# MonsieurETM/QPSK

Measured on AMD Instinct MI355X. Metric: complex Msamples/s demodulated + % HBM roofline, 2400-baud RRC+Costas path, higher is better.
Workload: dtype f32

## Files before the change

qpsk_amd/csrc/api.cpp:

```cpp
#include "../../include/qpsk_hip.h"
#include "host_math.h"
#include "kernels.h"

#include <hip/hip_runtime.h>
#include <limits.h>
#include <math.h>
#include <stdarg.h>
#include <stdio.h>
#include <stdlib.h>
#include <string.h>
#include <time.h>
#include <algorithm>
#include <map>
#include <vector>

using namespace qpsk;

static thread_local char g_err[512] = "";

static int fail(int code, const char *fmt, ...)
{
    va_list ap;
    va_start(ap, fmt);
    vsnprintf(g_err, sizeof g_err, fmt, ap);
// ... 8 lines not shown
            return fail(QPSK_ERR_HIP, "%s: %s (%s:%d)", #expr, hipGetErrorString(e_), __FILE__, __LINE__); \
    } while (0)

#define KERNEL_TRY(expr)                                                                      \
    do {                                                                                      \
        (void)hipGetLastError();  \
        int e_ = (expr);                                                                      \
        if (e_ != 0)                                                                          \
            return fail(QPSK_ERR_HIP, "%s: %s (%s:%d)", #expr, hipGetErrorString((hipError_t)e_), __FILE__, __LINE__); \
    } while (0)

struct DevBuf {
    void *p = nullptr;
    size_t cap = 0;
};

struct Tuning {
    int fused_g = -1, fused_s = -1, fused_lds = -1;
    int generic = -1;
    int pipe_nf = -1;
    int pipe_v = -1, pipe_g = -1;
    int layout_lo = -1, layout_hi = -1;
    int pipe_variant = -1;
    int hist_generic = -1;
    int fir_generic = -1;
    int stream_scan = -1;
    int stream_poll = -1;
    int stream_block = -1;
    int stream_carrier = -1;
    int lean_dma = -1;
    int hist_onepass = -1;
    int est_waves = -1;
    int lean_pair = -1;
    int viterbi_lds = -1;
    int fft_fused = -1;
    int viterbi_chunk_rows = -1;
};

static const struct { const char *name; int Tuning::*field; } TUNING_KEYS[] = {
    {"QPSK_FUSED_G", &Tuning::fused_g},       {"QPSK_FUSED_S", &Tuning::fused_s},     {"QPSK_FUSED_LDS", &Tuning::fused_lds},
    {"QPSK_FUSED_GENERIC", &Tuning::generic}, {"QPSK_PIPE_NF", &Tuning::pipe_nf},
    {"QPSK_PIPE_DBG", &Tuning::pipe_variant}, {"QPSK_HIST_GENERIC", &Tuning::hist_generic},
    {"QPSK_PIPE_V", &Tuning::pipe_v},         {"QPSK_PIPE_G", &Tuning::pipe_g},
    {"QPSK_PIPE_LAYOUT_LO", &Tuning::layout_lo}, {"QPSK_PIPE_LAYOUT_HI", &Tuning::layout_hi},
    {"QPSK_FIR_GENERIC", &Tuning::fir_generic}, {"QPSK_FFT_FUSED", &Tuning::fft_fused},
    {"QPSK_STREAM_BLOCK", &Tuning::stream_block}, {"QPSK_STREAM_POLL", &Tuning::stream_poll},
    {"QPSK_STREAM_SCAN", &Tuning::stream_scan}, {"QPSK_STREAM_CARRIER", &Tuning::stream_carrier},
    {"QPSK_LEAN_DMA", &Tuning::lean_dma},     {"QPSK_LEAN_PAIR", &Tuning::lean_pair},
    {"QPSK_EST_WAVES", &Tuning::est_waves},   {"QPSK_HIST_ONEPASS", &Tuning::hist_onepass},
    {"QPSK_VITERBI_LDS", &Tuning::viterbi_lds},   {"QPSK_VITERBI_CHUNK_ROWS", &Tuning::viterbi_chunk_rows},
};

#ifdef QPSK_PIPE_PROFILE
static const int PIPE_VARIANT_MASK = ~0;
#else
static const int PIPE_VARIANT_MASK = 4 | 8 | 16 | 64 | 128 | 256 | 512 | 1024 | 8192;
#endif

struct qpsk_ctx {
    int device = 0;
    Tuning tune;
    int ncu = 256;
    const char *last_kernel = "";
    int viterbi_launches = 0;
    bool taps_symmetric = false;
    hipStream_t stream = nullptr;
    qpsk_params prm{};
    int cycles = 0, nsym = 0;
    float taps[QPSK_NTAPS];
    float damping = 0.f, alpha = 0.f, beta = 0.f;
    float min_freq = 0.f, max_freq = 0.f;
    float *d_taps = nullptr;
    float *d_gains = nullptr;
    unsigned *h_done = nullptr, *d_done = nullptr;
    unsigned done_expect = 0;
    int *h_status = nullptr;
    int *d_status = nullptr;
    std::vector<float> h_gains;
    DevBuf index, filtered, mixed, keystream, sympad, mislist;
    DevBuf datacostas;
    DevBuf vitdec;
    DevBuf softgain;
// ... 512 lines not shown
            *d_index_out = (const int32_t *)c->index.p;
            return QPSK_OK;
        }
        const size_t bytes = sizeof(float) * 2 * (size_t)nframes * c->prm.frame_size;
        rc = ensure(c, c->filtered, bytes);
        if (rc) return rc;
        KERNEL_TRY(fir_full_rate(c, d_in, nullptr, (float *)c->filtered.p, nframes, c->prm.frame_size, pitch));
        KERNEL_TRY(launch_timing_hist((const float *)c->filtered.p, nframes, c->prm.frame_size, c->cycles,
                                      (int32_t *)c->index.p, nullptr, tuned(c->tune.hist_generic, 0) == 2, c->stream));
        *d_index_out = (const int32_t *)c->index.p;
        return QPSK_OK;
    }
    rc = fft_timing_indices(c, d_in, nframes, (int32_t *)c->index.p, nullptr, nullptr, pitch);
    if (rc) return rc;
    *d_index_out = (const int32_t *)c->index.p;
    return QPSK_OK;
}

struct ExtAcq {
    const int32_t *index;
    const float *seed;
};

static int rx_batch_common(qpsk_ctx *c, const float *d_in, long long frame_pitch, int nframes, int nbw, uint8_t *d_sym,
                           float *d_freq, float *d_phase, float *d_costas, int32_t *d_index, float *d_hz,
                           const ExtAcq *ext = nullptr, uint8_t *d_data = nullptr)
{
    if (!c || !d_in || !(d_sym || d_data)) return fail(QPSK_ERR_ARG, "qpsk_rx_batch: null context, input or symbol buffer");
    if (nframes <= 0) return fail(QPSK_ERR_ARG, "qpsk_rx_batch: nframes = %d", nframes);
    if (frame_pitch == 0) frame_pitch = c->prm.frame_size;
    if (frame_pitch < c->prm.frame_size)
        return fail(QPSK_ERR_ARG, "qpsk_rx_batch_pitched: frame_pitch %lld below frame_size %d", frame_pitch, c->prm.frame_size);
    if (bind(c)) return QPSK_ERR_HIP;
    const bool pipe_ok = c->cycles == pipe_cycles() && (c->prm.frame_size % 2) == 0 && (frame_pitch % 2) == 0 &&
                         ((uintptr_t)d_in % 16) == 0 && nbw * pipe_frames(1) <= 64 &&
                         tuned(c->tune.generic, 0) == 0;
    FusedArgs a{};
    a.x = reinterpret_cast<const float2 *>(d_in);
    a.frame_pitch = (size_t)frame_pitch;
    a.nframes = nframes;
    a.frame_size = c->prm.frame_size;
    a.cycles = c->cycles;
    a.nsym = c->nsym;
    pick_tiling(c, nframes, nbw, &a.G, &a.S);
    a.fixed_index = c->prm.fixed_index;
    a.dbg = tuned(c->tune.pipe_variant, 0) & PIPE_VARIANT_MASK;
    a.lean_dma = tuned(c->tune.lean_dma, 1) != 0;
    a.lean_twowin = tuned(c->tune.lean_dma, 1) != 2 ? 1 : 0;
    a.est_waves = tuned(c->tune.est_waves, 0);
    a.lean_pair = tuned(c->tune.lean_pair, 3);
    a.taps = c->d_taps;
    a.gains = c->d_gains;
    a.nbw = nbw;
    a.min_freq = c->min_freq;
    a.max_freq = c->max_freq;
    a.rs = c->prm.rs;
    a.sym = d_sym ? d_sym : d_data;
    a.data_rule = d_data && !d_sym;
    if (d_data && d_sym && !d_costas) {
        if (int rd = ensure(c, c->datacostas, sizeof(float2) * (size_t)nframes * (size_t)c->nsym)) return rd;
        d_costas = (float *)c->datacostas.p;
    }
    a.freq = d_freq;
    a.phase = d_phase;
    a.costas = reinterpret_cast<float2 *>(d_costas);
    a.hz = d_hz;
    a.status = c->d_status;
    const bool ext_index = ext && ext->index;
    if (ext && ext->seed) {
        a.state_in = ext->seed;
        a.seed_setters = 1;
    }

    enum { K_GENERIC, K_FUSED_PIPE, K_PIPE2, K_LEAN };
    struct Plan {
        int kind = K_GENERIC, nframes = 0, G = 0, nf = 0;
        unsigned long long layout = 0;
    };
    const int pipe_v = tuned(c->tune.pipe_v, nframes > 16 * c->ncu ? 2 : 1);
    auto plan_general = [&](int nfr, int pv, Plan *pl) -> int {
        pl->nframes = nfr;
        if (pipe_ok && pv == 2) {
            int G = (nfr + c->ncu - 1) / c->ncu;
            if (G > pipe2_max_frames()) G = pipe2_max_frames();
            G = tuned(c->tune.pipe_g, G);
            if (G > pipe2_max_frames()) G = pipe2_max_frames();
            if (G * nbw > 64) G = 64 / nbw;
            if (G < 1) G = 1;
            unsigned long long layout = 0;
            if (c->tune.layout_lo >= 0 || c->tune.layout_hi >= 0) {
                layout = ((unsigned long long)(unsigned)tuned(c->tune.layout_lo, 0) << 4) |
                         ((unsigned long long)(unsigned)tuned(c->tune.layout_hi, 0) << 24);
                int units = 0, nwin = 0;
                for (int w = 1; w < 16; w++) { const int cw = (int)((layout >> (4 * w)) & 15); units += cw; nwin += cw != 0; }
                if (units < 1 || (G + 1) / 2 != units || pipe2_lds_bytes(G, nwin, nbw) > (size_t)MAX_LDS_BYTES)
                    return fail(QPSK_ERR_ARG, "QPSK_PIPE_LAYOUT_*: %d units on %d waves do not match %d frames per workgroup", units, nwin, G);
            } else {
                for (;;) {
                    layout = pipe2_default_layout((G + 1) / 2);
                    int nwin = 0;
                    for (int w = 1; w < 16; w++) nwin += ((layout >> (4 * w)) & 15) != 0;
                    if (layout && pipe2_lds_bytes(G, nwin, nbw) <= (size_t)MAX_LDS_BYTES) break;
                    if (G == 1) return fail(QPSK_ERR_ARG, "pipeline geometry does not fit: %d loops per frame", nbw);
                    G--;
                }
            }
            pl->kind = K_PIPE2;
            pl->G = G;
            pl->layout = layout;
        } else if (pipe_ok) {
            auto fits = [&](int nf_) {
                return pipe_frames(nf_) * nbw <= 64 && pipe_lds_bytes(nf_, nbw) <= (size_t)MAX_LDS_BYTES;
            };
            const int full = pipe_max_nf();
            int nf = 1;
            while (nf < full && (long long)c->ncu * pipe_frames(nf) < nfr) nf++;
            nf = tuned(c->tune.pipe_nf, nf);
            if (nf < 1) nf = 1;
            if (nf > full) nf = full;
            while (nf > 1 && !fits(nf)) nf--;
            if (!fits(nf))
                return fail(QPSK_ERR_ARG, "pipeline geometry does not fit: nf %d, %d loops per frame", nf, nbw);
            pl->kind = K_FUSED_PIPE;
            pl->nf = nf;
        } else {
            pl->kind = K_GENERIC;
        }
        return QPSK_OK;
    };
    Plan main_pl, rem_pl;
    bool lean = false;
    if (pipe_ok && c->taps_symmetric && (pipe_v == 3 || c->tune.pipe_v < 0)) {
        int G = (nframes + c->ncu - 1) / c->ncu;
        G = tuned(c->tune.pipe_g, G);
        if (G > pipe2_max_frames()) G = pipe2_max_frames();
        G += G & 1;
        const bool wanted = pipe_v == 3 || G >= 4;
        unsigned long long layout = 0;
        if (c->tune.layout_lo >= 0 || c->tune.layout_hi >= 0)
            layout = ((unsigned long long)(unsigned)tuned(c->tune.layout_lo, 0) << 4) |
                     ((unsigned long long)(unsigned)tuned(c->tune.layout_hi, 0) << 24);
        else if (G >= 2)
// ... 67 lines not shown
    if (c->prm.timing_mode == QPSK_TIMING_FFT && !ext_index && rem_pl.nframes == 0 && nbw == 1 && tuned(c->tune.fft_fused, 1) != 0 &&
        c->prm.frame_size >= timing_fft_first() + timing_fft_nfft() &&
        ((main_pl.kind == K_FUSED_PIPE && main_pl.nf == pipe_max_nf() && !(tuned(c->tune.pipe_variant, 0) & (128 | 4))) ||
         (main_pl.kind == K_LEAN && lean_est_ok(a, main_pl.G, main_pl.layout)))) {
        int rt = fft_timing_tables(c, &est_tw, &est_cs);
        if (rt) return rt;
        fused_fft = true;
    }
    const int32_t *idx = nullptr;
    if (ext_index) {
        idx = ext->index;
    } else {
        int rc = timing_indices(c, d_in, (size_t)frame_pitch, nframes, &idx, fused_fft);
        if (rc) return rc;
    }
    a.index = idx;
    if (fused_fft) {
        a.est_tw = reinterpret_cast<const double2 *>(est_tw);
        a.est_cs = reinterpret_cast<const double2 *>(est_cs);
        a.index_out = d_index ? (int32_t *)c->index.p : nullptr;
        if (d_index) idx = (const int32_t *)c->index.p;
    }

    auto execute = [&](const FusedArgs &fa, const Plan &pl) -> int {
        if (fa.est_tw && !(pl.kind == K_FUSED_PIPE && pl.nf == pipe_max_nf()) && pl.kind != K_LEAN)
            return fail(QPSK_ERR_STATE, "internal: in-launch FFT timing estimate planned for a kernel that has none");
        if (fa.data_rule && pl.kind != K_LEAN)
            return fail(QPSK_ERR_STATE, "internal: data rule planned for a kernel that has none");
        switch (pl.kind) {
        case K_LEAN:
            KERNEL_TRY(launch_rx_lean(fa, pl.G, pl.layout, c->d_status, c->stream));
            c->last_kernel = fa.est_tw ? "rx_lean_kernel (FFT timing estimate inside the launch)" : "rx_lean_kernel";
            break;
        case K_PIPE2:
            KERNEL_TRY(launch_rx_pipe2(fa, pl.G, pl.layout, c->d_status, c->stream));
            c->last_kernel = "rx_pipe2_kernel";
            break;
        case K_FUSED_PIPE:
            KERNEL_TRY(launch_rx_fused_pipe(fa, pl.nf, c->d_status, c->stream));
            c->last_kernel = fa.est_tw ? "rx_fused_pipe_kernel (FFT timing estimate inside the launch)" : "rx_fused_pipe_kernel";
            break;
        default:
            KERNEL_TRY(launch_rx_fused(fa, c->stream));
            c->last_kernel = "rx_fused_kernel";
        }
        return QPSK_OK;
    };
    {
        FusedArgs am = a;
        am.nframes = main_pl.nframes;
        int rc2 = execute(am, main_pl);
        if (rc2) return rc2;
        if (rem_pl.nframes > 0) {
            FusedArgs ar = a;
            const size_t o = (size_t)main_pl.nframes;
            ar.nframes = rem_pl.nframes;
            ar.x += o * a.frame_pitch;
            if (ar.index) ar.index += o;
            if (ar.state_in) ar.state_in += 2 * o * (size_t)nbw;
            ar.sym += o * (size_t)a.nsym;
            if (ar.freq) ar.freq += o;
            if (ar.phase) ar.phase += o;
            if (ar.hz) ar.hz += o;
            const char *lk = c->last_kernel;
            rc2 = execute(ar, rem_pl);
            if (rc2) return rc2;
            c->last_kernel = lk;
        }
    }
    if (hist_mode && !ext && c->d_hint && idx && tuned(c->tune.hist_onepass, -1) != 0) {
// ... 1314 lines not shown
```

qpsk_amd/csrc/kernels.h:

```cpp
#ifndef QPSK_KERNELS_H
#define QPSK_KERNELS_H

#include <hip/hip_runtime.h>
#include <stddef.h>
#include <stdint.h>

namespace qpsk {

constexpr int LOOKBACK = 128;
constexpr int LOOKAHEAD = 8;
constexpr int MAX_LDS_BYTES = 160 * 1024;
constexpr int MAX_INDEX = 7;
constexpr int STATUS_PIPE_TIMEOUT = 1;
constexpr int STATUS_PHASE_RANGE = 2;
constexpr int STATUS_NONFINITE = 3;
constexpr int STATUS_BAD_INDEX = 4;
constexpr int STATUS_EST_NONFINITE = 5;
constexpr int STATUS_SOFT_NONFINITE = 6;
constexpr int STATUS_SOFT_BAD_LAG = 7;

struct FusedArgs {
    const float2 *x;
    size_t frame_pitch;
    int nframes, frame_size, cycles, nsym;
    int G, S;
    int mixed;
    int share_simd0;
    const int32_t *index;
    int fixed_index;
    const double2 *est_tw, *est_cs;
    int32_t *index_out;
    int lean_twowin;
    int lean_dma;
    int est_waves;
    int lean_pair;
    int dbg;
    const float2 *dsrc;
    int dstride;
    const float2 *refill;
    float2 *refill_dst;
    int refill_planar;
    const int32_t *frame_list, *frame_list_count;
    const float *taps;
    const float *gains;
    int nbw;
    float min_freq, max_freq;
    double rs;
    const float *state_in;
    int seed_setters;
    float *state_out;
    uint8_t *sym;
    uint8_t *sym_pad;
    float *freq, *phase;
    float2 *costas;
    float *hz;
    int *status;
    float *carrier_state;
    float2 *carrier_tab;
    int carrier_frame;
    int data_rule;
};

size_t fused_lds_bytes(int G, int S, int cycles, int nbw);
int prepare_kernels(void);
int launch_rx_fused(const FusedArgs &a, hipStream_t s);
size_t pipe_lds_bytes(int NF, int nbw);
int pipe_frames(int NF);
int pipe_cycles(void);
int pipe_max_nf(void);
int prepare_pipe_kernel(void);
int launch_rx_fused_pipe(const FusedArgs &a, int NF, int *status, hipStream_t s);
int launch_costas_pipe(const FusedArgs &a, int NF, int *status, hipStream_t s);
size_t pipe2_lds_bytes(int G, int nwin, int nbw);
int pipe2_max_fir(void);
int pipe2_max_frames(void);
int pipe2_max_units_per_wave(void);
int pipe2_max_hw_waves(void);
unsigned long long pipe2_default_layout(int NU);
int launch_rx_pipe2(const FusedArgs &a, int G, unsigned long long layout, int *status, hipStream_t s);
size_t lean_lds_bytes(int G, int nwin);
unsigned long long lean_default_layout(int NU);
bool lean_shape_ok(const FusedArgs &a, int G);
int launch_rx_lean(const FusedArgs &a, int G, unsigned long long layout, int *status, hipStream_t s);
bool lean_est_ok(const FusedArgs &a, int G, unsigned long long layout);
bool rx_hist_shape_ok(const FusedArgs &a);
int launch_rx_hist(const FusedArgs &a, int32_t *index_true, const int32_t *hint, int32_t *mis_list, int32_t *mis_count, int *status, hipStream_t s);
int launch_index_majority(const int32_t *index, int nframes, int32_t *hint, int32_t *mis_count, int32_t *h_stats, hipStream_t s);
int launch_rrc_fir(const float *x, const float *memory, float *y, const float *taps, int nframes, int length,
                   hipStream_t s, size_t in_pitch = 0);
int launch_rrc_fir_stream(const float *x, const float *memory, float *y, const float *taps, int nframes, int length,
                          hipStream_t s, size_t in_pitch = 0, int ncu = 0);
int launch_delay_line(const float *x, float *memory, int nframes, int length, hipStream_t s);
int launch_rrc_fir_fast(const float *x, const float *memory, float *y, const float *H, const float *tw, int nframes, int length,
                        hipStream_t s);
int rrc_fir_fast_hop(void);
int rrc_fir_fast_nfft(void);
int launch_timing_hist(const float *y, int nframes, int frame_size, int cycles, int32_t *index, int32_t *hist,
                       bool generic, hipStream_t s);
int launch_costas(const float *d, int nframes, int nsym, int dstride, int nbw, const float *gains, float min_freq,
                  float max_freq, const float *state_in, float *state_out, uint8_t *sym, float *costas, int *status,
                  hipStream_t s);
int launch_decimate(const float *filtered, const int32_t *index, float *dec, int nstreams, int frame_size,
                    int cycles, int nsym, hipStream_t s);
int launch_mixer(const int16_t *pcm, float *out, float *state, int nstreams, int frame_size, hipStream_t s);
int launch_fft(const double *in, double *out, const double *tw, int nbatch, int n, int log2n, int inverse,
               hipStream_t s);
int fft_lds_max_n(void);
int fft_big_block(void);
int launch_fft_big(const double *in, double *out, const double *twb, const double *twn, int nbatch, int n, int log2n,
                   int inverse, hipStream_t s);
size_t timing_scan_lds_bytes(void);
int timing_scan_tile(void);
// ... 155 lines not shown
```

qpsk_amd/csrc/rx_fused.hip:

```cpp
#include <hip/hip_runtime.h>
#include <stdint.h>
#include "qpsk_device.h"
#include "costas_asm.h"
#include "costas_asm_lo.h"
#include "fir_full8s_asm.h"
#include "fir_r2_asm.h"
#include "fir_r4_asm.h"
#include "fir_lean_asm.h"
#include "fir_lean_data_asm.h"
#include "fir_full8_asm.h"
#include "timing_fft_wave.h"
#include "carrier.h"
#ifdef QPSK_PIPE_PROFILE
#include "fir_lean_prof_asm.h"
#endif
#include "kernels.h"

#ifndef QPSK_PIPE1_ASM
#define QPSK_PIPE1_ASM 1
#endif

namespace qpsk {

static_assert(FIR_R2_ASM_END_VGPR <= 168, "rx_pipe2_kernel: three FIR waves per SIMD");
// ... 73 lines not shown
__device__ __forceinline__ void report_status(int *status, int what)
{
    __hip_atomic_store(status, what, __ATOMIC_RELAXED, __HIP_MEMORY_SCOPE_SYSTEM);
}

__device__ __forceinline__ bool wait_ge(int *p, int target, int *abort_flag)
{
    int spins = 0;
    while (ld_acquire(p) < target) {
        __builtin_amdgcn_s_sleep(2);
        if (++spins > SPIN_LIMIT || __hip_atomic_load(abort_flag, __ATOMIC_RELAXED, __HIP_MEMORY_SCOPE_WORKGROUP)) {
            __hip_atomic_store(abort_flag, 1, __ATOMIC_RELAXED, __HIP_MEMORY_SCOPE_WORKGROUP);
            return false;
        }
    }
    return true;
}

}

using namespace pipe;

struct StreamHi {
    template <class... A> static __device__ __forceinline__ void ring(A &&...a) { costas_asm_run_ring(a...); }
    template <class... A> static __device__ __forceinline__ void ring_pair(A &&...a) { costas_asm_run_ring_pair(a...); }
    template <class... A> static __device__ __forceinline__ unsigned run(A &&...a) { return costas_asm_run(a...); }
};
struct StreamLo {
    template <class... A> static __device__ __forceinline__ void ring(A &&...a) { costas_asm_run_ring_lo(a...); }
    template <class... A> static __device__ __forceinline__ void ring_pair(A &&...a) { costas_asm_run_ring_pair_lo(a...); }
    template <class... A> static __device__ __forceinline__ unsigned run(A &&...a) { return costas_asm_run_lo(a...); }
};

template <class GM, class ST = StreamHi, class SM>
__device__ __forceinline__ void costas_wave(const FusedArgs &a, SM *sm, const float2 *dring, float *zring, int G,
                                            int f0, int lane, int nchunks, int *status)
{
    QPSK_GEOM_CONSTANTS(GM);
    const int nbw = a.nbw, N = a.nsym;
    if (a.share_simd0 != ((a.dbg & 512) != 0)) __builtin_amdgcn_s_setprio(1);
    else __builtin_amdgcn_s_setprio(3);
    const bool pair = a.lean_pair != 0;
    const bool odd = pair && (lane & 1);
    const int g = pair ? lane >> 1 : lane / nbw, b = pair ? 0 : lane - g * nbw;
    const bool inwg = pair ? lane < 2 * G : lane < G * nbw;
    const bool active = inwg && f0 + g < a.nframes;
    Loop st = {0.0f, 0.0f};
    LoopGains lg = {0.0f, 0.0f, a.min_freq, a.max_freq};
    bool over = false;
    if (active) {
        lg.alpha = a.gains[2 * b];
        lg.beta = a.gains[2 * b + 1];
        if (a.state_in) {
            st.phase = a.state_in[2 * ((size_t)(f0 + g) * nbw + b)];
            st.freq = a.state_in[2 * ((size_t)(f0 + g) * nbw + b) + 1];
            if (a.seed_setters) seed_setters(st.phase, st.freq, a.min_freq, a.max_freq, over);
        }
    }
    const int gl = inwg ? g : 0;
    const int gw = a.mixed == 2 ? gl / 2 : a.mixed == 1 && gl >= 12 ? 3 + (gl - 12) / 2 : gl / FWV;
    const float2 *dl = dring + (size_t)gl * DSTRIDE;
    float *zl = zring + (size_t)(pair ? gl : lane) * ZSTRIDE;
    const bool fast_clamp = a.min_freq < 0.0f && a.max_freq > 0.0f;
    float ph = st.phase, fr = st.freq;
    auto zero_run = [&](int from, int to) {
        const uint4 *p = reinterpret_cast<const uint4 *>(dl + from);
        unsigned acc = 0;
        for (int i = 0; i < (to - from) / 2; i++) {
            const uint4 v = p[i];
            acc |= v.x | v.y | v.z | v.w;
        }
        return acc == 0u;
    };
    auto excusable = [&](unsigned long long lanes, int from, int to) {
        const bool z = ((lanes >> lane) & 1ull) != 0ull && __float_as_uint(ph) != 0x80000000u && __float_as_uint(fr) != 0x80000000u &&
                       zero_run(from, to);
        return (unsigned long long)__ballot(z);
    };
    const float al = lg.alpha, be = lg.beta, fmin_ = a.min_freq, fmax_ = a.max_freq;
    bool ok = true;
#ifdef QPSK_PIPE_PROFILE
    const bool cprof = (a.dbg & 32) && blockIdx.x == 0;
    unsigned long long cw = 0, cs = 0, ct = 0;
    auto ctick = [&](unsigned long long &acc) {
        if (cprof) {
            unsigned long long t;
            asm volatile("s_memtime %0\n\ts_waitcnt lgkmcnt(0)" : "=s"(t)::"memory");
            acc += t - ct;
            ct = t;
        }
    };
    unsigned long long dummy = 0;
    ctick(dummy);
#endif
#ifdef QPSK_PIPE_PROFILE
// ... 157 lines not shown
        if (lane == 0) st_release(&sm->consumed, c + 1);
#ifdef QPSK_PIPE_PROFILE
        ctick(cs);
#endif
    }
#ifdef QPSK_PIPE_PROFILE
    if (cprof && lane == 0 && !ring_prof)
        printf("serial wave: %d chunks; cycles per chunk: wait for the FIR waves %llu, steps %llu\n", nchunks, cw / nchunks, cs / nchunks);
    if (timeline) {
        if (lane == 0 && blockIdx.x < 1024) {
            unsigned long long *tl = g_timeline + 48 * blockIdx.x;
            tl[1] = rp_rt0; tl[2] = rp_rt1; tl[3] = rp_rt2; tl[4] = rp_real();
        }
    } else if (ring_prof && lane == 0)
        printf("wg %3d serial wave: %d chunks, %llu entries into the stream; cycles per chunk inside the stream %llu (= %llu per step), "
               "outside it (waiting for the FIR waves, redone groups) %llu; wall time (100 MHz clock): wave start -> first step %.2f us, "
               "first -> last step %.2f us\n", (int)blockIdx.x, nchunks, rp_calls, rp_in / nchunks,
               rp_in / nchunks / S, rp_out / nchunks, (double)(rp_rt1 - rp_rt0) * 0.01, (double)(rp_rt2 - rp_rt1) * 0.01);
#endif
    st.phase = ph; st.freq = fr;
    if (active && ok && !odd) {
        const size_t o = (size_t)(f0 + g) * nbw + b;
        if (a.freq) a.freq[o] = st.freq;
        if (a.phase) a.phase[o] = st.phase;
        if (a.hz) a.hz[o] = (float)((double)st.freq * a.rs / TAU);
        if (a.state_out) { a.state_out[2 * o] = st.phase; a.state_out[2 * o + 1] = st.freq; }
    }
    if (!ok && lane == 0) report_status(status, STATUS_PIPE_TIMEOUT);
    if (over) report_status(status, STATUS_PHASE_RANGE);
    else if (active && ok && !loop_state_finite(ph, fr)) report_status(status, STATUS_NONFINITE);
}

template <class GM, int RW = GM::R, bool DATA = false>
__device__ __forceinline__ void flush_records(const FusedArgs &a, const float *zring, const float2 *dring, int g, int frame,
                                              int q, int chunk, uint8_t *sym_row = nullptr)
{
    constexpr int DSTRIDE = GM::DSTRIDE;
    constexpr int R = RW, S = GM::S, ZSTRIDE = GM::ZSTRIDE;
    static_assert(R == 2 || R == 4, "packs 2 or 4 symbols per store");
    const int nbw = a.nbw, N = a.nsym;
    const int slot = (chunk % DR) * S, sym0 = chunk * S;
    const int cnt = min(S, N - sym0);
    for (int b = 0; b < nbw; b++) {
        const int row = g * nbw + b;
        const size_t o = ((size_t)frame * nbw + b) * N + sym0 + R * q;
        float2 z[R];
        uint32_t packed = 0;
        float phv[R];
        float2 dv[R];
        {
            const float *zp = zring + (size_t)row * ZSTRIDE + slot + R * q;
            const float2 *dp = dring + (size_t)g * DSTRIDE + slot + R * q;
            if constexpr (R == 4) {
                const float4 p4 = *reinterpret_cast<const float4 *>(zp);
                const float4 da = reinterpret_cast<const float4 *>(dp)[0], db = reinterpret_cast<const float4 *>(dp)[1];
                phv[0] = p4.x; phv[1] = p4.y; phv[2] = p4.z; phv[3] = p4.w;
                dv[0] = make_float2(da.x, da.y); dv[1] = make_float2(da.z, da.w);
                dv[2] = make_float2(db.x, db.y); dv[3] = make_float2(db.z, db.w);
            } else {
                const float2 p2 = *reinterpret_cast<const float2 *>(zp);
                const float4 da = *reinterpret_cast<const float4 *>(dp);
                phv[0] = p2.x; phv[1] = p2.y;
                dv[0] = make_float2(da.x, da.y); dv[1] = make_float2(da.z, da.w);
            }
        }
#pragma unroll
        for (int r = 0; r < R; r++)
            z[r] = derotate<false>(phv[r], dv[r]);
        if (chunk == 0 && q == 0)
            z[0] = derotate<true>(phv[0], dv[0]);
#pragma unroll
        for (int r = 0; r < R; r++)
            packed |= (uint32_t)(DATA ? data_rule(z[r]) : slicer(z[r])) << (8 * r);
        if (a.sym) {
            uint8_t *so = sym_row ? sym_row + sym0 + R * q : a.sym + o;
            if (R * q + R <= cnt && ((N | sym0) & (R - 1)) == 0) {
                if constexpr (R == 4) *reinterpret_cast<uint32_t *>(so) = packed;
                else *reinterpret_cast<uint16_t *>(so) = (uint16_t)packed;
            } else {
                for (int r = 0; r < R; r++)
                    if (R * q + r < cnt) so[r] = (uint8_t)(packed >> (8 * r));
            }
        }
        if (a.costas) {
            for (int r = 0; r < R; r++)
                if (R * q + r < cnt) a.costas[o + r] = z[r];
        }
    }
}

__global__ void __launch_bounds__(64 * (GeomNarrow::MAX_NF + 2))
costas_pipe_kernel(FusedArgs a, int *status)
{
    using GM = GeomNarrow;
    QPSK_GEOM_CONSTANTS(GM);
    static_assert(R == 2 || R == 4, "flush_records packs 2 or 4 symbols per store");
    extern __shared__ __attribute__((aligned(16))) unsigned char smem_raw[];
    Smem *sm = reinterpret_cast<Smem *>(smem_raw);
    const int NF = (int)blockDim.x / 64 - 1 - (a.carrier_state ? 1 : 0);
    const int G = NF * FWV;
    float2 *dring = reinterpret_cast<float2 *>(smem_raw + sizeof(Smem));
    float *zring = reinterpret_cast<float *>(dring + (size_t)G * DSTRIDE);
    const int tid = threadIdx.x, wave = tid >> 6, lane = tid & 63;
    const int N = a.nsym;
    const int f0 = blockIdx.x * G;
    const int nchunks = (N + S - 1) / S;
    if (tid < MAX_WAVES) sm->ready[tid] = 0;
    if (tid == 0) { sm->consumed = 0; sm->abort_flag = 0; }
    __syncthreads();

    if (wave == 0) {
        costas_wave<GM>(a, sm, dring, zring, G, f0, lane, nchunks, status);
        return;
    }
    if (wave == NF + 1) {
        if (blockIdx.x == 0 && lane == 0)
            carrier_block(a.carrier_state, a.carrier_tab, a.carrier_frame, carrier_split(a.carrier_frame), a.carrier_frame / 2);
        return;
    }
    const int w = wave - 1;
    const int fl = lane / QL, q = lane % QL;
// ... 405 lines not shown
#define QPSK_PIPE2_MAXFIR 9
#ifndef QPSK_PIPE2_ASM
#define QPSK_PIPE2_ASM 1
#endif
#ifndef QPSK_PIPE2_DEPTH
#define QPSK_PIPE2_DEPTH 1
#endif
namespace pipe2 {
constexpr int QL = 32, R = 2, UF = 2;
constexpr int S = GeomNarrow::S, CH = S * C;
constexpr int PAD = R * C, PADS = 2;
constexpr int TSTEPS = NTAPS + C * (R - 1);
constexpr int NLD = CH / 128;
constexpr int BLK = 128 + PADS * (128 / PAD);
constexpr int WS = 720;
__device__ __host__ constexpr int slot_of(int p) { return p + PADS * (p / PAD); }
constexpr int MAX_UNITS = 16, MAX_FIR = QPSK_PIPE2_MAXFIR, MAX_UW = (MAX_UNITS + MAX_FIR - 1) / MAX_FIR;
constexpr int MAX_THREADS = 64 * (MAX_FIR + 1 + (MAX_FIR - 1) / 3);
static_assert(S == QL * R && CH % 128 == 0 && slot_of(CH + HIST - 1) < WS && WS % 2 == 0 && PAD % 2 == 0 &&
              PAD * (QL - 1) + TSTEPS - 1 <= CH + HIST - 1 - (C - 1), "window geometry: every position a lane reads is written for every index < C");
static_assert(MAX_UNITS <= MAX_WAVES, "one ready[] counter per unit");

struct Unit {
    int u;
    bool fv[UF], all_valid;
    const float4 *src[UF];
    int ix[UF];
    float4 hist[UF];
};
}

template <int NUW>
__device__ __forceinline__ void fir_wave2(const FusedArgs &a, Smem *sm, float2 *mywin, float2 *dring, float *zring, int G,
                                          int widx, int u0, int f0, int lane, int nchunks, int *status)
{
    constexpr int nuw = NUW;
    using namespace pipe2;
    using GM = GeomNarrow;
    constexpr int DSTRIDE = GM::DSTRIDE;
    const int L = a.frame_size;
    const int fl = lane / QL, q = lane % QL;
    const bool simd0 = ((threadIdx.x >> 6) & 3) == 0;
    const float4 *taps4 = reinterpret_cast<const float4 *>(sm->taps);
    const float2 *rd = mywin + fl * WS + (PAD + PADS) * q;

    Unit un[NUW];
#pragma unroll
    for (int ui = 0; ui < NUW; ui++) {
        Unit &U = un[ui];
        U.u = u0 + ui;
        U.all_valid = UF * U.u + UF <= G && f0 + UF * U.u + UF <= a.nframes;
#pragma unroll
        for (int ff = 0; ff < UF; ff++) {
            const int fr = f0 + UF * U.u + ff;
            U.fv[ff] = UF * U.u + ff < G && fr < a.nframes;
            const int ix = checked_index(a.index ? (U.fv[ff] ? a.index[fr] : 0) : a.fixed_index, a.status);
            U.ix[ff] = __builtin_amdgcn_readfirstlane(ix);
            U.src[ff] = reinterpret_cast<const float4 *>(a.x + (size_t)(U.fv[ff] ? fr : 0) * a.frame_pitch);
            U.hist[ff] = make_float4(0.0f, 0.0f, 0.0f, 0.0f);
        }
    }

    auto prefetch = [&](const Unit &U, float4 (&pre)[UF][NLD], int c) {
        if (U.all_valid && (c + 1) * CH <= L) {
#pragma unroll
            for (int ff = 0; ff < UF; ff++)
#pragma unroll
                for (int j = 0; j < NLD; j++)
// ... 101 lines not shown
                        v2f pa0, pa1, pb0, pb1;
                        if constexpr (a0) pa0 = va * tg[tb % NG][u];
                        if constexpr (a1) pa1 = va * tg[(tb - 1 + NG) % NG][u];
                        if constexpr (b0) pb0 = vb * tg[tb % NG][u + 1];
                        if constexpr (b1) pb1 = vb * tg[(tb - 1 + NG) % NG][u + 1];
                        if constexpr (a0 && a1 && b0 && b1) {
                            asm volatile("" : "+v"(pa0), "+v"(pa1), "+v"(pb0), "+v"(pb1));
                        } else {
                            if constexpr (a0) asm volatile("" : "+v"(pa0));
                            if constexpr (a1) asm volatile("" : "+v"(pa1));
                            if constexpr (b0) asm volatile("" : "+v"(pb0));
                            if constexpr (b1) asm volatile("" : "+v"(pb1));
                        }
                        if constexpr (a0) ac[0] = ac[0] + pa0;
                        if constexpr (a1) ac[1] = ac[1] + pa1;
                        if constexpr (b0) ac[0] = ac[0] + pb0;
                        if constexpr (b1) ac[1] = ac[1] + pb1;
                        asm volatile("" : "+v"(ac[0]), "+v"(ac[1]));
                    }
                });
            });
#endif
        } else {
            ac[0] = v2f{0.7f, 0.3f}; ac[1] = v2f{0.7f, 0.3f};
        }
        tick(3);
        const int g = UF * U.u + fl, frame = f0 + g;
        const bool mine = g < G && frame < a.nframes;
        if (c >= DR) {
            if (!wait_ge(&sm->consumed, c - DR + 1, &sm->abort_flag)) return false;
            tick(0);
            int gf = g, qf = q;
            asm volatile("" : "+v"(gf), "+v"(qf));
            if (mine) flush_records<GM, R>(a, zring, dring, gf, f0 + gf, qf, c - DR);
            tick(1);
        }
        if (g < G) {
            const float2 s0 = fir_gain(make_float2(ac[0].x, ac[0].y)), s1 = fir_gain(make_float2(ac[1].x, ac[1].y));
            int gr = g, qr = q;
            asm volatile("" : "+v"(gr), "+v"(qr));
            *reinterpret_cast<float4 *>(dring + (size_t)gr * DSTRIDE + (c % DR) * S + R * qr) = make_float4(s0.x, s0.y, s1.x, s1.y);
        }
        if (lane == 0) st_release(&sm->ready[U.u], c + 1);
        tick(4);
        return true;
    };

    float4 pre[UF][NLD];
    prefetch(un[0], pre, 0);
    bool ok = true;
    tick(-1);
    for (int c = 0; c < nchunks && ok; c++) {
        static_for<0, NUW>([&](auto uic) {
            constexpr int ui = decltype(uic)::value, nx = (ui + 1) % NUW;
            constexpr bool last_unit = ui + 1 == NUW;
            if (ok) ok = run_unit(un[ui], pre, c, un[nx], !last_unit || c + 1 < nchunks, last_unit ? c + 1 : c);
        });
    }
    if (ok) {
        ok = wait_ge(&sm->consumed, nchunks, &sm->abort_flag);
        if (ok)
#pragma unroll
            for (int ui = 0; ui < NUW; ui++) {
                const int g = UF * (u0 + ui) + fl, frame = f0 + g;
                for (int c = max(0, nchunks - DR); c < nchunks; c++)
                    if (g < G && frame < a.nframes) flush_records<GM, R>(a, zring, dring, g, frame, q, c);
            }
    }
    if (!ok && lane == 0) report_status(status, STATUS_PIPE_TIMEOUT);
#ifdef QPSK_PIPE_PROFILE
    if (prof && lane == 0)
        printf("FIR wave %d (%d units): %d chunks; cycles per chunk: wait for the loop %llu, flush %llu, window staging %llu, "
               "filter %llu, ring hand-over %llu\n", widx, nuw, nchunks, tacc[0] / nchunks, tacc[1] / nchunks, tacc[2] / nchunks,
               tacc[3] / nchunks, tacc[4] / nchunks);
#endif
}

__global__ void __launch_bounds__(pipe2::MAX_THREADS)
rx_pipe2_kernel(FusedArgs a, unsigned long long layout, int nwin, int *status)
{
    using namespace pipe2;
    using GM = GeomNarrow;
    extern __shared__ __attribute__((aligned(16))) unsigned char smem_raw[];
    Smem *sm = reinterpret_cast<Smem *>(smem_raw);
    const int G = a.G;
    float2 *win = reinterpret_cast<float2 *>(smem_raw + sizeof(Smem));
    float2 *dring = win + (size_t)nwin * UF * WS;
    float *zring = reinterpret_cast<float *>(dring + (size_t)G * GM::DSTRIDE);
    const int tid = threadIdx.x, lane = tid & 63;
    const int wave = __builtin_amdgcn_readfirstlane(tid >> 6);
    const int f0 = blockIdx.x * G;
    const int nchunks = (a.nsym + S - 1) / S;

    for (int i = tid; i < 128; i += blockDim.x)
        sm->taps[i] = i < NTAPS ? a.taps[i] : 0.0f;
    if (tid < MAX_WAVES) sm->ready[tid] = 0;
    if (tid == 0) { sm->consumed = 0; sm->abort_flag = 0; }
    __syncthreads();

    if (wave == 0) {
        costas_wave<GM>(a, sm, dring, zring, G, f0, lane, nchunks, status);
        return;
    }
    const int mine = (int)((layout >> (4 * wave)) & 15);
    if (mine == 0) return;
    int u0 = 0, widx = 0;
    for (int v = 1; v < wave; v++) {
        const int cv = (int)((layout >> (4 * v)) & 15);
        u0 += cv;
        widx += cv != 0;
    }
    float2 *mywin = win + (size_t)widx * UF * WS;
    if (mine == 2)
        fir_wave2<2>(a, sm, mywin, dring, zring, G, widx, u0, f0, lane, nchunks, status);
    else
        fir_wave2<1>(a, sm, mywin, dring, zring, G, widx, u0, f0, lane, nchunks, status);
}

size_t pipe2_lds_bytes(int G, int nwin, int nbw)
{
    using GM = GeomNarrow;
    size_t b = sizeof(Smem) + sizeof(float2) * ((size_t)nwin * pipe2::UF * pipe2::WS + (size_t)G * GM::DSTRIDE) +
               sizeof(float) * (size_t)G * nbw * GM::ZSTRIDE;
    return (b + 15) & ~(size_t)15;
}

int pipe2_max_fir(void) { return pipe2::MAX_FIR; }
int pipe2_max_frames(void) { return pipe2::UF * pipe2::MAX_UNITS; }
int pipe2_max_units_per_wave(void) { return pipe2::MAX_UW; }
int pipe2_max_hw_waves(void) { return pipe2::MAX_THREADS / 64; }

unsigned long long pipe2_default_layout(int NU)
{
    using namespace pipe2;
    int cnt[16] = {0};
    const int hwmax = MAX_THREADS / 64;
    const bool share = NU > 8 && MAX_UW == 2;
    int left = NU;
    for (int round = 0; round < MAX_UW && left > 0; round++)
        for (int w = 1; w < hwmax && left > 0; w++) {
            if ((w & 3) == 0 && !(share && w == 4)) continue;
            if (share && (w == 11 || (round == 1 && w > 7))) continue;
            cnt[w]++;
            left--;
        }
    unsigned long long layout = 0;
    for (int w = 1; w < hwmax; w++) layout |= (unsigned long long)cnt[w] << (4 * w);
    return left == 0 ? layout : 0;
}

int launch_rx_pipe2(const FusedArgs &a0, int G, unsigned long long layout, int *status, hipStream_t s)
{
    using namespace pipe2;
    if (a0.est_tw) return (int)hipErrorInvalidValue;
    FusedArgs a = a0;
    const int NU = (G + UF - 1) / UF;
    int units = 0, nwin = 0, hw = 1;
    for (int w = 1; w < 16; w++) {
        const int cw = (int)((layout >> (4 * w)) & 15);
        if (cw > MAX_UW || (cw && w >= MAX_THREADS / 64)) return (int)hipErrorInvalidValue;
        units += cw;
        nwin += cw != 0;
        if (cw) hw = w + 1;
    }
    if (G < 1 || G > UF * MAX_UNITS || G * a.nbw > 64 || units != NU || (layout & 15) ||
        pipe2_lds_bytes(G, nwin, a.nbw) > (size_t)MAX_LDS_BYTES)
        return (int)hipErrorInvalidValue;
    a.G = G;
    a.lean_pair = 0;
    a.mixed = 2;
    a.share_simd0 = ((layout >> 16) & 15) != 0 || ((layout >> 32) & 15) != 0;
    const int blocks = (a.nframes + G - 1) / G;
    hipLaunchKernelGGL(rx_pipe2_kernel, dim3(blocks), dim3(64 * hw), pipe2_lds_bytes(G, nwin, a.nbw), s, a, layout, nwin, status);
    return (int)hipGetLastError();
}

namespace lean {
constexpr int PRM_DWORDS = 20;
constexpr int HW_WAVES = pipe2::MAX_THREADS / 64;
constexpr int WS = WS_LEAN_SLOTS;
struct Ctl {
    int ready[MAX_WAVES];
    int consumed;
    int abort_flag;
    int pad_[2];
};
struct GeomLean : GeomNarrow {
    static constexpr int DSTRIDE = 194;
    static constexpr int ZSTRIDE = 388;
};
constexpr int ROW_BYTES = 1552, Z_OFFSET_BYTES = 1024;
static_assert(GeomLean::DSTRIDE * 8 == ROW_BYTES && GeomLean::ZSTRIDE * 4 == ROW_BYTES &&
              Z_OFFSET_BYTES == DR * GeomNarrow::S * 8 && Z_OFFSET_BYTES + DR * GeomNarrow::S * 4 <= ROW_BYTES &&
              ROW_BYTES % 16 == 0 && (ROW_BYTES / 4) % 64 == 4, "ring rows: symbols, records, bank spread");
static_assert(sizeof(Ctl) % 16 == 0 && offsetof(Ctl, ready) == 0 && offsetof(Ctl, consumed) == 64 &&
              offsetof(Ctl, abort_flag) == 68, "fir_lean_asm.h addresses the counters by these offsets");
static_assert(PRM_DWORDS * 4 <= ROW_BYTES - Z_OFFSET_BYTES, "a parameter block fits the record half of a row");
static_assert(FIR_LEAN_END_VGPR <= 168, "three waves per SIMD");
static_assert(FIR_LEAN_WOFF == sizeof(float2) * pipe2::UF * WS, "fir_lean_loop2_dma2w: unit 1's window follows unit 0's");
static_assert(WS % 2 == 0 && pipe2::slot_of(pipe2::PAD * (pipe2::QL - 1) + pipe2::TSTEPS - 1) < WS &&
              pipe2::slot_of(pipe2::CH + HIST - 1) < WS + 16, "window: every position a lane reads, and a frame's spill stays in the next frame's history slots");
__device__ __host__ constexpr int rows_of(int G) { return G > HW_WAVES ? G : HW_WAVES; }
}
constexpr size_t LEAN_EST_LDS_BYTES = 128 * sizeof(float) + 32 * sizeof(int);

__device__ __forceinline__ uint8_t *lean_unit_rows(const FusedArgs &a, int f0, int u)
// ... 731 lines not shown
```

Baseline: 446,400.

## Pair lanes per Costas loop and split bandwidths across FIR waves in pipe2

Adds a pipe2 planning path for multi-bandwidth runs that gives each Costas loop two lanes (lean_pair) and, when only one FIR unit exists, splits the per-bandwidth loops across up to three FIR waves. Each of those waves has its own decimated-sample ring and flushes only its slice of bandwidths. The aim is more parallelism per workgroup and less serial FIR/flush work when there are few frames per block. In exchange it uses more LDS for the duplicated rings, adds more waves, and makes the Costas lane indexing more complex.

```diff
diff --git a/qpsk_amd/csrc/api.cpp b/qpsk_amd/csrc/api.cpp
--- a/qpsk_amd/csrc/api.cpp
+++ b/qpsk_amd/csrc/api.cpp
@@ -64,6 +64,7 @@
     int hist_onepass = -1;
     int est_waves = -1;
     int lean_pair = -1;
+    int bw_split = -1;
     int viterbi_lds = -1;
     int fft_fused = -1;
     int viterbi_chunk_rows = -1;
@@ -80,6 +81,7 @@
     {"QPSK_STREAM_SCAN", &Tuning::stream_scan}, {"QPSK_STREAM_CARRIER", &Tuning::stream_carrier},
     {"QPSK_LEAN_DMA", &Tuning::lean_dma},     {"QPSK_LEAN_PAIR", &Tuning::lean_pair},
     {"QPSK_EST_WAVES", &Tuning::est_waves},   {"QPSK_HIST_ONEPASS", &Tuning::hist_onepass},
+    {"QPSK_BW_SPLIT", &Tuning::bw_split},
     {"QPSK_VITERBI_LDS", &Tuning::viterbi_lds},   {"QPSK_VITERBI_CHUNK_ROWS", &Tuning::viterbi_chunk_rows},
 };
 
@@ -658,9 +660,9 @@
     if (frame_pitch < c->prm.frame_size)
         return fail(QPSK_ERR_ARG, "qpsk_rx_batch_pitched: frame_pitch %lld below frame_size %d", frame_pitch, c->prm.frame_size);
     if (bind(c)) return QPSK_ERR_HIP;
-    const bool pipe_ok = c->cycles == pipe_cycles() && (c->prm.frame_size % 2) == 0 && (frame_pitch % 2) == 0 &&
-                         ((uintptr_t)d_in % 16) == 0 && nbw * pipe_frames(1) <= 64 &&
-                         tuned(c->tune.generic, 0) == 0;
+    const bool pipe_shape_ok = c->cycles == pipe_cycles() && (c->prm.frame_size % 2) == 0 && (frame_pitch % 2) == 0 &&
+                               ((uintptr_t)d_in % 16) == 0 && tuned(c->tune.generic, 0) == 0;
+    const bool pipe_ok = pipe_shape_ok && nbw * pipe_frames(1) <= 64;
     FusedArgs a{};
     a.x = reinterpret_cast<const float2 *>(d_in);
     a.frame_pitch = (size_t)frame_pitch;
@@ -702,38 +704,60 @@
     struct Plan {
         int kind = K_GENERIC, nframes = 0, G = 0, nf = 0;
         unsigned long long layout = 0;
+        bool pair = false;
+        int split = 1;
     };
     const int pipe_v = tuned(c->tune.pipe_v, nframes > 16 * c->ncu ? 2 : 1);
+    auto plan_pipe2 = [&](int nfr, int gcap, bool quiet, Plan *pl) -> int {
+        int G = (nfr + c->ncu - 1) / c->ncu;
+        if (G > pipe2_max_frames()) G = pipe2_max_frames();
+        G = tuned(c->tune.pipe_g, G);
+        if (G > pipe2_max_frames()) G = pipe2_max_frames();
+        if (G > gcap) G = gcap;
+        if (G < 1) G = 1;
+        unsigned long long layout = 0;
+        if (c->tune.layout_lo >= 0 || c->tune.layout_hi >= 0) {
+            layout = ((unsigned long long)(unsigned)tuned(c->tune.layout_lo, 0) << 4) |
+                     ((unsigned long long)(unsigned)tuned(c->tune.layout_hi, 0) << 24);
+            int units = 0, nwin = 0;
+            for (int w = 1; w < 16; w++) { const int cw = (int)((layout >> (4 * w)) & 15); units += cw; nwin += cw != 0; }
+            if (units < 1 || (G + 1) / 2 != units || pipe2_lds_bytes(G, nwin, nbw) > (size_t)MAX_LDS_BYTES)
+                return quiet ? 1 : fail(QPSK_ERR_ARG, "QPSK_PIPE_LAYOUT_*: %d units on %d waves do not match %d frames per workgroup", units, nwin, G);
+        } else {
+            for (;;) {
+                layout = pipe2_default_layout((G + 1) / 2);
+                int nwin = 0;
+                for (int w = 1; w < 16; w++) nwin += ((layout >> (4 * w)) & 15) != 0;
+                if (layout && pipe2_lds_bytes(G, nwin, nbw) <= (size_t)MAX_LDS_BYTES) break;
+                if (G == 1) return quiet ? 1 : fail(QPSK_ERR_ARG, "pipeline geometry does not fit: %d loops per frame", nbw);
+                G--;
+            }
+        }
+        pl->kind = K_PIPE2;
+        pl->nframes = nfr;
+        pl->G = G;
+        pl->layout = layout;
+        return QPSK_OK;
+    };
     auto plan_general = [&](int nfr, int pv, Plan *pl) -> int {
         pl->nframes = nfr;
+        if (nbw > 1 && 2 * nbw <= 64 && pipe_shape_ok && tuned(c->tune.lean_pair, 3) != 0 && c->tune.pipe_v != 1) {
+            Plan pp;
+            if (plan_pipe2(nfr, 32 / nbw, true, &pp) == QPSK_OK && 2 * pp.G * nbw <= 64 && (nfr + pp.G - 1) / pp.G <= c->ncu) {
+                *pl = pp;
+                pl->pair = true;
+                if ((pp.G + 1) / 2 == 1 && pp.layout == 0x10ull) {
+                    int K = tuned(c->tune.bw_split, 3);
+                    if (K > 3) K = 3;
+                    if (K > nbw) K = nbw;
+                    while (K > 1 && ((K - 1) * ((nbw + K - 1) / K) >= nbw || pipe2_lds_bytes(pp.G, K, nbw, K) > (size_t)MAX_LDS_BYTES)) K--;
+                    pl->split = K < 1 ? 1 : K;
+                }
+                return QPSK_OK;
+            }
+        }
         if (pipe_ok && pv == 2) {
-            int G = (nfr + c->ncu - 1) / c->ncu;
-            if (G > pipe2_max_frames()) G = pipe2_max_frames();
-            G = tuned(c->tune.pipe_g, G);
-            if (G > pipe2_max_frames()) G = pipe2_max_frames();
-            if (G * nbw > 64) G = 64 / nbw;
-            if (G < 1) G = 1;
-            unsigned long long layout = 0;
-            if (c->tune.layout_lo >= 0 || c->tune.layout_hi >= 0) {
-                layout = ((unsigned long long)(unsigned)tuned(c->tune.layout_lo, 0) << 4) |
-                         ((unsigned long long)(unsigned)tuned(c->tune.layout_hi, 0) << 24);
-                int units = 0, nwin = 0;
-                for (int w = 1; w < 16; w++) { const int cw = (int)((layout >> (4 * w)) & 15); units += cw; nwin += cw != 0; }
-                if (units < 1 || (G + 1) / 2 != units || pipe2_lds_bytes(G, nwin, nbw) > (size_t)MAX_LDS_BYTES)
-                    return fail(QPSK_ERR_ARG, "QPSK_PIPE_LAYOUT_*: %d units on %d waves do not match %d frames per workgroup", units, nwin, G);
-            } else {
-                for (;;) {
-                    layout = pipe2_default_layout((G + 1) / 2);
-                    int nwin = 0;
-                    for (int w = 1; w < 16; w++) nwin += ((layout >> (4 * w)) & 15) != 0;
-                    if (layout && pipe2_lds_bytes(G, nwin, nbw) <= (size_t)MAX_LDS_BYTES) break;
-                    if (G == 1) return fail(QPSK_ERR_ARG, "pipeline geometry does not fit: %d loops per frame", nbw);
-                    G--;
-                }
-            }
-            pl->kind = K_PIPE2;
-            pl->G = G;
-            pl->layout = layout;
+            return plan_pipe2(nfr, 64 / nbw, false, pl);
         } else if (pipe_ok) {
             auto fits = [&](int nf_) {
                 return pipe_frames(nf_) * nbw <= 64 && pipe_lds_bytes(nf_, nbw) <= (size_t)MAX_LDS_BYTES;
@@ -867,10 +891,13 @@
             KERNEL_TRY(launch_rx_lean(fa, pl.G, pl.layout, c->d_status, c->stream));
             c->last_kernel = fa.est_tw ? "rx_lean_kernel (FFT timing estimate inside the launch)" : "rx_lean_kernel";
             break;
-        case K_PIPE2:
-            KERNEL_TRY(launch_rx_pipe2(fa, pl.G, pl.layout, c->d_status, c->stream));
-            c->last_kernel = "rx_pipe2_kernel";
+        case K_PIPE2: {
+            FusedArgs fp = fa;
+            fp.lean_pair = pl.pair ? 1 : 0;
+            KERNEL_TRY(launch_rx_pipe2(fp, pl.G, pl.layout, c->d_status, c->stream, pl.split));
+            c->last_kernel = pl.pair ? "rx_pipe2_kernel, two lanes per loop" : "rx_pipe2_kernel";
             break;
+        }
         case K_FUSED_PIPE:
             KERNEL_TRY(launch_rx_fused_pipe(fa, pl.nf, c->d_status, c->stream));
             c->last_kernel = fa.est_tw ? "rx_fused_pipe_kernel (FFT timing estimate inside the launch)" : "rx_fused_pipe_kernel";
diff --git a/qpsk_amd/csrc/kernels.h b/qpsk_amd/csrc/kernels.h
--- a/qpsk_amd/csrc/kernels.h
+++ b/qpsk_amd/csrc/kernels.h
@@ -34,6 +34,7 @@
     int lean_dma;
     int est_waves;
     int lean_pair;
+    int bw_split, bw_block;
     int dbg;
     const float2 *dsrc;
     int dstride;
@@ -71,13 +72,13 @@
 int prepare_pipe_kernel(void);
 int launch_rx_fused_pipe(const FusedArgs &a, int NF, int *status, hipStream_t s);
 int launch_costas_pipe(const FusedArgs &a, int NF, int *status, hipStream_t s);
-size_t pipe2_lds_bytes(int G, int nwin, int nbw);
+size_t pipe2_lds_bytes(int G, int nwin, int nbw, int nshare = 1);
 int pipe2_max_fir(void);
 int pipe2_max_frames(void);
 int pipe2_max_units_per_wave(void);
 int pipe2_max_hw_waves(void);
 unsigned long long pipe2_default_layout(int NU);
-int launch_rx_pipe2(const FusedArgs &a, int G, unsigned long long layout, int *status, hipStream_t s);
+int launch_rx_pipe2(const FusedArgs &a, int G, unsigned long long layout, int *status, hipStream_t s, int bw_split = 1);
 size_t lean_lds_bytes(int G, int nwin);
 unsigned long long lean_default_layout(int NU);
 bool lean_shape_ok(const FusedArgs &a, int G);
diff --git a/qpsk_amd/csrc/rx_fused.hip b/qpsk_amd/csrc/rx_fused.hip
--- a/qpsk_amd/csrc/rx_fused.hip
+++ b/qpsk_amd/csrc/rx_fused.hip
@@ -129,7 +129,7 @@
     template <class... A> static __device__ __forceinline__ unsigned run(A &&...a) { return costas_asm_run_lo(a...); }
 };
 
-template <class GM, class ST = StreamHi, class SM>
+template <class GM, class ST = StreamHi, bool BW = false, class SM>
 __device__ __forceinline__ void costas_wave(const FusedArgs &a, SM *sm, const float2 *dring, float *zring, int G,
                                             int f0, int lane, int nchunks, int *status)
 {
@@ -139,8 +139,9 @@
     else __builtin_amdgcn_s_setprio(3);
     const bool pair = a.lean_pair != 0;
     const bool odd = pair && (lane & 1);
-    const int g = pair ? lane >> 1 : lane / nbw, b = pair ? 0 : lane - g * nbw;
-    const bool inwg = pair ? lane < 2 * G : lane < G * nbw;
+    const int row = BW ? (pair ? lane >> 1 : lane) : lane;
+    const int g = BW ? row / nbw : pair ? lane >> 1 : lane / nbw, b = BW ? row - g * nbw : pair ? 0 : lane - g * nbw;
+    const bool inwg = BW ? row < G * nbw : pair ? lane < 2 * G : lane < G * nbw;
     const bool active = inwg && f0 + g < a.nframes;
     Loop st = {0.0f, 0.0f};
     LoopGains lg = {0.0f, 0.0f, a.min_freq, a.max_freq};
@@ -155,9 +156,10 @@
         }
     }
     const int gl = inwg ? g : 0;
-    const int gw = a.mixed == 2 ? gl / 2 : a.mixed == 1 && gl >= 12 ? 3 + (gl - 12) / 2 : gl / FWV;
-    const float2 *dl = dring + (size_t)gl * DSTRIDE;
-    float *zl = zring + (size_t)(pair ? gl : lane) * ZSTRIDE;
+    const int share = BW && a.bw_split > 1 && inwg ? b / a.bw_block : 0;
+    const int gw = BW ? share * ((G + 1) / 2) + gl / 2 : a.mixed == 2 ? gl / 2 : a.mixed == 1 && gl >= 12 ? 3 + (gl - 12) / 2 : gl / FWV;
+    const float2 *dl = dring + (size_t)(BW ? share * G + gl : gl) * DSTRIDE;
+    float *zl = zring + (size_t)(BW ? row : pair ? gl : lane) * ZSTRIDE;
     const bool fast_clamp = a.min_freq < 0.0f && a.max_freq > 0.0f;
     float ph = st.phase, fr = st.freq;
     auto zero_run = [&](int from, int to) {
@@ -381,8 +383,8 @@
 }
 
 template <class GM, int RW = GM::R, bool DATA = false>
-__device__ __forceinline__ void flush_records(const FusedArgs &a, const float *zring, const float2 *dring, int g, int frame,
-                                              int q, int chunk, uint8_t *sym_row = nullptr)
+__device__ __forceinline__ void flush_records_range(const FusedArgs &a, const float *zring, const float2 *dring, int g, int frame,
+                                                    int q, int chunk, uint8_t *sym_row, int b0, int b1)
 {
     constexpr int DSTRIDE = GM::DSTRIDE;
     constexpr int R = RW, S = GM::S, ZSTRIDE = GM::ZSTRIDE;
@@ -390,7 +392,7 @@
     const int nbw = a.nbw, N = a.nsym;
     const int slot = (chunk % DR) * S, sym0 = chunk * S;
     const int cnt = min(S, N - sym0);
-    for (int b = 0; b < nbw; b++) {
+    for (int b = b0; b < b1; b++) {
         const int row = g * nbw + b;
         const size_t o = ((size_t)frame * nbw + b) * N + sym0 + R * q;
         float2 z[R];
@@ -436,6 +438,13 @@
                 if (R * q + r < cnt) a.costas[o + r] = z[r];
         }
     }
+}
+
+template <class GM, int RW = GM::R, bool DATA = false>
+__device__ __forceinline__ void flush_records(const FusedArgs &a, const float *zring, const float2 *dring, int g, int frame,
+                                              int q, int chunk, uint8_t *sym_row = nullptr)
+{
+    flush_records_range<GM, RW, DATA>(a, zring, dring, g, frame, q, chunk, sym_row, 0, a.nbw);
 }
 
 __global__ void __launch_bounds__(64 * (GeomNarrow::MAX_NF + 2))
@@ -907,8 +916,9 @@
 
 template <int NUW>
 __device__ __forceinline__ void fir_wave2(const FusedArgs &a, Smem *sm, float2 *mywin, float2 *dring, float *zring, int G,
-                                          int widx, int u0, int f0, int lane, int nchunks, int *status)
-{
+                                          int widx, int u0, int f0, int lane, int nchunks, int *status, int r0 = 0, int b0 = 0, int b1 = -1)
+{
+    if (b1 < 0) b1 = a.nbw;
     constexpr int nuw = NUW;
     using namespace pipe2;
     using GM = GeomNarrow;
@@ -1076,7 +1086,7 @@
             tick(0);
             int gf = g, qf = q;
             asm volatile("" : "+v"(gf), "+v"(qf));
-            if (mine) flush_records<GM, R>(a, zring, dring, gf, f0 + gf, qf, c - DR);
+            if (mine) flush_records_range<GM, R>(a, zring, dring, gf, f0 + gf, qf, c - DR, nullptr, b0, b1);
             tick(1);
         }
         if (g < G) {
@@ -1085,7 +1095,7 @@
             asm volatile("" : "+v"(gr), "+v"(qr));
             *reinterpret_cast<float4 *>(dring + (size_t)gr * DSTRIDE + (c % DR) * S + R * qr) = make_float4(s0.x, s0.y, s1.x, s1.y);
         }
-        if (lane == 0) st_release(&sm->ready[U.u], c + 1);
+        if (lane == 0) st_release(&sm->ready[r0 + U.u], c + 1);
         tick(4);
         return true;
     };
@@ -1108,7 +1118,7 @@
             for (int ui = 0; ui < NUW; ui++) {
                 const int g = UF * (u0 + ui) + fl, frame = f0 + g;
                 for (int c = max(0, nchunks - DR); c < nchunks; c++)
-                    if (g < G && frame < a.nframes) flush_records<GM, R>(a, zring, dring, g, frame, q, c);
+                    if (g < G && frame < a.nframes) flush_records_range<GM, R>(a, zring, dring, g, frame, q, c, nullptr, b0, b1);
             }
     }
     if (!ok && lane == 0) report_status(status, STATUS_PIPE_TIMEOUT);
@@ -1129,8 +1139,9 @@
     Smem *sm = reinterpret_cast<Smem *>(smem_raw);
     const int G = a.G;
     float2 *win = reinterpret_cast<float2 *>(smem_raw + sizeof(Smem));
+    const int nshare = a.bw_split > 1 ? a.bw_split : 1;
     float2 *dring = win + (size_t)nwin * UF * WS;
-    float *zring = reinterpret_cast<float *>(dring + (size_t)G * GM::DSTRIDE);
+    float *zring = reinterpret_cast<float *>(dring + (size_t)nshare * G * GM::DSTRIDE);
     const int tid = threadIdx.x, lane = tid & 63;
     const int wave = __builtin_amdgcn_readfirstlane(tid >> 6);
     const int f0 = blockIdx.x * G;
@@ -1143,28 +1154,39 @@
     __syncthreads();
 
     if (wave == 0) {
-        costas_wave<GM>(a, sm, dring, zring, G, f0, lane, nchunks, status);
+        costas_wave<GM, StreamHi, true>(a, sm, dring, zring, G, f0, lane, nchunks, status);
         return;
     }
-    const int mine = (int)((layout >> (4 * wave)) & 15);
-    if (mine == 0) return;
-    int u0 = 0, widx = 0;
-    for (int v = 1; v < wave; v++) {
-        const int cv = (int)((layout >> (4 * v)) & 15);
-        u0 += cv;
-        widx += cv != 0;
+    int mine, u0 = 0, widx = 0, r0 = 0, b0 = 0, b1 = a.nbw;
+    float2 *myring = dring;
+    if (nshare > 1) {
+        if (wave > nshare) return;
+        mine = 1;
+        widx = wave - 1;
+        r0 = widx * ((G + UF - 1) / UF);
+        b0 = widx * a.bw_block;
+        b1 = min(a.nbw, b0 + a.bw_block);
+        myring = dring + (size_t)widx * G * GM::DSTRIDE;
+    } else {
+        mine = (int)((layout >> (4 * wave)) & 15);
+        if (mine == 0) return;
+        for (int v = 1; v < wave; v++) {
+            const int cv = (int)((layout >> (4 * v)) & 15);
+            u0 += cv;
+            widx += cv != 0;
+        }
     }
     float2 *mywin = win + (size_t)widx * UF * WS;
     if (mine == 2)
         fir_wave2<2>(a, sm, mywin, dring, zring, G, widx, u0, f0, lane, nchunks, status);
     else
-        fir_wave2<1>(a, sm, mywin, dring, zring, G, widx, u0, f0, lane, nchunks, status);
-}
-
-size_t pipe2_lds_bytes(int G, int nwin, int nbw)
+        fir_wave2<1>(a, sm, mywin, myring, zring, G, widx, u0, f0, lane, nchunks, status, r0, b0, b1);
+}
+
+size_t pipe2_lds_bytes(int G, int nwin, int nbw, int nshare)
 {
     using GM = GeomNarrow;
-    size_t b = sizeof(Smem) + sizeof(float2) * ((size_t)nwin * pipe2::UF * pipe2::WS + (size_t)G * GM::DSTRIDE) +
+    size_t b = sizeof(Smem) + sizeof(float2) * ((size_t)nwin * pipe2::UF * pipe2::WS + (size_t)nshare * G * GM::DSTRIDE) +
                sizeof(float) * (size_t)G * nbw * GM::ZSTRIDE;
     return (b + 15) & ~(size_t)15;
 }
@@ -1193,7 +1215,7 @@
     return left == 0 ? layout : 0;
 }
 
-int launch_rx_pipe2(const FusedArgs &a0, int G, unsigned long long layout, int *status, hipStream_t s)
+int launch_rx_pipe2(const FusedArgs &a0, int G, unsigned long long layout, int *status, hipStream_t s, int bw_split)
 {
     using namespace pipe2;
     if (a0.est_tw) return (int)hipErrorInvalidValue;
@@ -1207,15 +1229,21 @@
         nwin += cw != 0;
         if (cw) hw = w + 1;
     }
+    const int K = bw_split > 1 ? bw_split : 1, block = (a.nbw + K - 1) / K;
+    if (K > 1 && (NU != 1 || K > 3 || (K - 1) * block >= a.nbw || layout != 0x10ull)) return (int)hipErrorInvalidValue;
+    if (K > 1) { nwin = K; hw = K + 1; }
     if (G < 1 || G > UF * MAX_UNITS || G * a.nbw > 64 || units != NU || (layout & 15) ||
-        pipe2_lds_bytes(G, nwin, a.nbw) > (size_t)MAX_LDS_BYTES)
+        pipe2_lds_bytes(G, nwin, a.nbw, K) > (size_t)MAX_LDS_BYTES)
         return (int)hipErrorInvalidValue;
+    a.bw_split = K;
+    a.bw_block = block;
+    if (a.lean_pair && (a.nbw < 2 || 2 * G * a.nbw > 64)) return (int)hipErrorInvalidValue;
     a.G = G;
-    a.lean_pair = 0;
+    a.lean_pair = a.lean_pair != 0;
     a.mixed = 2;
     a.share_simd0 = ((layout >> 16) & 15) != 0 || ((layout >> 32) & 15) != 0;
     const int blocks = (a.nframes + G - 1) / G;
-    hipLaunchKernelGGL(rx_pipe2_kernel, dim3(blocks), dim3(64 * hw), pipe2_lds_bytes(G, nwin, a.nbw), s, a, layout, nwin, status);
+    hipLaunchKernelGGL(rx_pipe2_kernel, dim3(blocks), dim3(64 * hw), pipe2_lds_bytes(G, nwin, a.nbw, K), s, a, layout, nwin, status);
     return (int)hipGetLastError();
 }
 
```

Result: no change. 446,900 (median of 2 runs) (+0.1%).
